# HJReachability/ilqgames

Hardware: AMD Instinct MI355X
Metric: iLQ iterations/sec (batch) (higher is better)
Workload: dtype f64

## Files before the change

### ilqgames_amd/csrc/ilqg_models.hpp

```cpp
#pragma once

#include "ilqg_common.hpp"
#include "ilqg_trig.hpp"

namespace ilqg {

template <typename T> __device__ __forceinline__ T t_sin(T x);
template <> __device__ __forceinline__ float t_sin<float>(float x) { return sinf(x); }
template <> __device__ __forceinline__ double t_sin<double>(double x) { return sin(x); }
template <typename T> __device__ __forceinline__ T t_cos(T x);
template <> __device__ __forceinline__ float t_cos<float>(float x) { return cosf(x); }
template <> __device__ __forceinline__ double t_cos<double>(double x) { return cos(x); }
template <typename T> __device__ __forceinline__ T t_tan(T x);
template <> __device__ __forceinline__ float t_tan<float>(float x) { return tanf(x); }
template <> __device__ __forceinline__ double t_tan<double>(double x) { return tan(x); }
template <typename T> __device__ __forceinline__ T t_sqrt(T x);
template <> __device__ __forceinline__ float t_sqrt<float>(float x) { return sqrtf(x); }
template <> __device__ __forceinline__ double t_sqrt<double>(double x) { return sqrt(x); }
template <typename T> __device__ __forceinline__ T t_hypot(T x, T y);
template <> __device__ __forceinline__ float t_hypot<float>(float x, float y) { return hypotf(x, y); }
template <> __device__ __forceinline__ double t_hypot<double>(double x, double y) { return hypot(x, y); }
template <typename T> __device__ __forceinline__ T t_abs(T x) { return x < T(0) ? -x : x; }

__device__ __forceinline__ bool is_unicycle(int kind) {
// ... 110 lines not shown
    xd[0] = L * t_cos(x[2]);
    xd[1] = L * t_sin(x[2]);
    xd[2] = x[3];
    xd[3] = u0;
    xd[4] = xd[5] = xd[6] = xd[7] = T(0);
  } else {
    sub_eval<T>(kind, L, x, u0, u1, xd, d0, d1);
    xd[6] = xd[7] = T(0);
  }
}
template <typename T>
__device__ __forceinline__ void sub_integrate8(int kind, T L, double interval, T* x, T u0, T u1, T d0 = T(0),
                                               T d1 = T(0)) {
  constexpr int XS = kSubStatesMax;
  const T h = T(interval / 2.0);
#pragma unroll 1
  for (int s = 0; s < 2; s++) {
    T k1[XS], k2[XS], k3[XS], k4[XS], xt[XS];
    sub_eval8(kind, L, x, u0, u1, k1, d0, d1);
#pragma unroll
    for (int i = 0; i < XS; i++) { k1[i] = h * k1[i]; xt[i] = x[i] + T(0.5) * k1[i]; }
    sub_eval8(kind, L, xt, u0, u1, k2, d0, d1);
#pragma unroll
    for (int i = 0; i < XS; i++) { k2[i] = h * k2[i]; xt[i] = x[i] + T(0.5) * k2[i]; }
    sub_eval8(kind, L, xt, u0, u1, k3, d0, d1);
#pragma unroll
    for (int i = 0; i < XS; i++) { k3[i] = h * k3[i]; xt[i] = x[i] + k3[i]; }
    sub_eval8(kind, L, xt, u0, u1, k4, d0, d1);
#pragma unroll
    for (int i = 0; i < XS; i++) {
      k4[i] = h * k4[i];
      x[i] += (k1[i] + T(2.0) * (k2[i] + k3[i]) + k4[i]) / T(6.0);
    }
  }
}

template <typename T> __device__ __forceinline__ void t_sincos(T x, T* s, T* c);
template <> __device__ __forceinline__ void t_sincos<float>(float x, float* s, float* c) { sincosf(x, s, c); }
template <> __device__ __forceinline__ void t_sincos<double>(double x, double* s, double* c) { sincos(x, s, c); }

template <typename T>
__device__ __forceinline__ T div_by(T x, T c, T rc) {
  const T q = x * rc;
  const T r = __builtin_fma(-q, c, x);
  return __builtin_fma(r, rc, q);
}
__device__ __forceinline__ float div_by(float x, float c, float rc) {
  const float q = x * rc;
  const float r = __builtin_fmaf(-q, c, x);
  return __builtin_fmaf(r, rc, q);
}

#pragma clang fp contract(off)
template <typename T, bool DIST = false, bool DUB = false>
__device__ __forceinline__ void sub_integrate_stages(int kind, T L, double interval, T* x, T u0, T u1, int q, int lane,
                                                     T* gth, bool any_car, T d0 = T(0), T d1 = T(0),
                                                     unsigned long long group = ~0ull) {
  const T h = T(interval / 2.0);
  const T six = T(6.0), rsix = T(1.0) / T(6.0), rL = T(1.0) / L;
  const bool dubins = DUB && kind == ILQG_DYN_DUBINS_CAR;
  const bool car = DIST ? false : (kind == ILQG_DYN_CAR_5D || kind == ILQG_DYN_CAR_6D);
  const bool car6 = car && kind == ILQG_DYN_CAR_6D;
  const int j = q & 3;
  const bool s1 = q >= 4;
  const T aj = j == 0 ? T(0) : (j == 3 ? T(1) : T(0.5));
  const T cq = aj + (s1 ? T(1) : T(0));
  const T ang0 = car ? x[3] : x[2];
  const T hk = h * u0;
  const T ang_q = t_fma(cq, hk, ang0);
  const T ang_end = t_fma(T(2), hk, ang0);
  const T v0 = car ? x[4] : x[3];
  const T hj = h * u1;
  T v_q, v_end, a_end = T(0);
  {
    const T a0 = x[5];
    const T a_1 = a0 + hj;
    const T v_1 = t_fma(T(0.5) * h, hj, t_fma(h, a0, v0));
    const T vb = s1 ? v_1 : v0, ab = s1 ? a_1 : a0;
    const T bj = j == 2 ? T(0.25) : (j == 3 ? T(0.5) : T(0));
    const T v6_q = t_fma(bj * h, hj, t_fma(aj * h, ab, vb));
    const T v6_end = t_fma(T(0.5) * h, hj, t_fma(h, a_1, v_1));
    const T v5_q = t_fma(cq, hj, v0), v5_end = t_fma(T(2), hj, v0);
    v_q = car6 ? v6_q : v5_q;
    v_end = car6 ? v6_end : v5_end;
    a_end = t_fma(T(2), hj, a0);
    if (dubins) v_q = L;
  }
  T th_q = ang_q, th_end = ang_end;
  if (any_car) {
    const T kth = car ? h * (div_by(v_q, L, rL) * fast_tan(ang_q, group)) : T(0);
    gth[lane] = kth;
    lds_sync(true);
    const T* g = gth + (lane & ~7);
    const T k0 = g[0], k1 = g[1], k2 = g[2], k3 = g[3], k4 = g[4], k5 = g[5], k6 = g[6], k7 = g[7];
    const T kprev = (lane & 7) ? gth[lane - 1] : T(0);
    const T th1 = x[2] + div_by(t_fma(T(2), k1 + k2, k0) + k3, six, rsix);
    const T th2 = th1 + div_by(t_fma(T(2), k5 + k6, k4) + k7, six, rsix);
    const T thb = s1 ? th1 : x[2];
    th_q = car ? t_fma(aj, kprev, thb) : ang_q;
    th_end = car ? th2 : ang_end;
  }
  T sn, cs;
  fast_sincos(th_q, &sn, &cs, group);
  const T kx = DIST ? h * t_fma(v_q, cs, d0) : h * (v_q * cs);
  const T ky = DIST ? h * t_fma(v_q, sn, d1) : h * (v_q * sn);
  T* gxy = gth + 64;
  gxy[2 * lane] = kx;
  gxy[2 * lane + 1] = ky;
  lds_sync(true);
  const T* gq = gxy + 2 * (lane & ~7);
  T px = x[0], py = x[1];
#pragma unroll
  for (int s = 0; s < 2; s++) {
    const T a1 = gq[8 * s + 0], b1 = gq[8 * s + 1], a2 = gq[8 * s + 2], b2 = gq[8 * s + 3];
    const T a3 = gq[8 * s + 4], b3 = gq[8 * s + 5], a4 = gq[8 * s + 6], b4 = gq[8 * s + 7];
    px += div_by(t_fma(T(2), a2 + a3, a1) + a4, six, rsix);
    py += div_by(t_fma(T(2), b2 + b3, b1) + b4, six, rsix);
  }
  x[0] = px;
  x[1] = py;
  x[2] = th_end;
  if (car) {
    x[3] = ang_end;
    x[4] = v_end;
    if (car6) x[5] = a_end;
  } else if (!dubins) {
    x[3] = v_end;
  }
}

template <typename T>
__device__ __forceinline__ T stage_value(T v) {
  asm volatile("" : "+v"(v));
  return v;
}

template <typename T, bool DUB = false>
__device__ __forceinline__ void sub_integrate_stages_seq(int kind, T L, double interval, T* x, T u0, T u1) {
  const T h = T(interval / 2.0);
  const T six = T(6.0), rsix = T(1.0) / T(6.0), rL = T(1.0) / L;
  const bool dubins = DUB && kind == ILQG_DYN_DUBINS_CAR;
  const bool car = kind == ILQG_DYN_CAR_5D || kind == ILQG_DYN_CAR_6D;
  const bool car6 = car && kind == ILQG_DYN_CAR_6D;
  const T ang0 = car ? x[3] : x[2];
  const T hk = h * u0;
  const T ang_end = t_fma(T(2), hk, ang0);
  const T v0 = car ? x[4] : x[3];
  const T hj = h * u1;
  const T a0 = x[5];
  const T a_1 = a0 + hj;
  const T v_1 = t_fma(T(0.5) * h, hj, t_fma(h, a0, v0));
  const T v6_end = t_fma(T(0.5) * h, hj, t_fma(h, a_1, v_1));
  const T v5_end = t_fma(T(2), hj, v0);
  const T v_end = car6 ? v6_end : v5_end;
  const T a_end = t_fma(T(2), hj, a0);
  T ang[8], vq[8], kth[8];
// ... 748 lines not shown
```

### ilqgames_amd/csrc/ilqg_solve.hpp

```cpp
#pragma once
#ifndef ILQG_ROLL_PRIO
#define ILQG_ROLL_PRIO 1
#endif

#include "ilqg_lq.hpp"
#include "ilqg_lq_openloop.hpp"
#include "ilqg_lq_feedback2.hpp"
#include "ilqg_lq_feedback1w.hpp"
#include "ilqg_lq_generic.hpp"
#include "ilqg_stages.hpp"

namespace ilqg {

template <typename T>
struct SolveArgs {
  const T* x0;
  T *xs, *us;
  T *P, *alpha;
  T* total_costs;
  int *iters, *status, *converged;
  const int* active;
  T* ws;
  size_t ws_stride;
  int fixed_iters;
// ... 610 lines not shown
    s = state_load<T>(w, L);
  }
  return s;
}

template <typename T>
__device__ __forceinline__ void trial_rollout_args(const SolveArgs<T>& sa, const InstanceBuffers<T>& ib, int b, int n,
                                                   SolveState<T>& s, RolloutArgs<T>& ra) {
  const int snew = 1 - s.sacc;
  ra.x0 = s.initial ? sa.x0 + size_t(b) * n : ib.XS(s.cur);
  ra.xs_ref = s.initial ? ib.XS(0) : ib.XS(s.cur);
  ra.us_ref = s.initial ? ib.US(0) : ib.US(s.cur);
  ra.P = s.initial ? ib.PB(0) : ib.PB(snew);
  ra.alpha = s.initial ? ib.AL(0) : ib.AL(snew);
  ra.alpha_scale = s.initial ? T(1) : s.step;
  ra.xs = s.initial ? ib.XS(1) : ib.XS(1 - s.cur);
  ra.us = s.initial ? ib.US(1) : ib.US(1 - s.cur);
  if (s.initial) {
    s.cur = 1;
    s.qmode = Q_COSTS;
  } else {
    s.qmode = sa.prm.linesearch ? Q_TRIAL : Q_LIN;
  }
}

template <typename T, int NX, int NP, int MU>
__device__ __forceinline__ void roll_pair_instances(const DevProblem& p, const SolveArgs<T>& sa, int b0, int b1, T* sm) {
  constexpr int n = NX, N = NP, m = NP * MU;
  const InstanceBuffers<T> ib0(p, sa, b0), ib1(p, sa, b1 < 0 ? b0 : b1);
  SolveState<T> s0, s1;
  RolloutArgs<T> r0, r1;
  auto enter = [&](const InstanceBuffers<T>& ib, int b, SolveState<T>& s, RolloutArgs<T>& r) -> bool {
    if (b < 0) return false;
    if (!sa.first) {
      if (reinterpret_cast<const SolveState<T>*>(ib.w + ib.L.state)->stage != ST_ROLLOUT) return false;
    } else if (sa.active && !sa.active[b]) {
      if (threadIdx.x == 0) reinterpret_cast<SolveState<T>*>(ib.w + ib.L.state)->stage = ST_DONE;
      return false;
    }
    s = trial_state_begin<T>(p, sa, ib, b, n, N, m);
    if (s.stage != ST_ROLLOUT) return false;
    trial_rollout_args<T>(sa, ib, b, n, s, r);
    r.iv = instance_values(p, b);
    return true;
  };
  const bool g0 = enter(ib0, b0, s0, r0), g1 = enter(ib1, b1, s1, r1);
  if (!g0 && !g1) return;
  __syncthreads();
  rollout_pair<T, NX, NP * MU, (MU == 1)>(p, g0 ? r0 : r1, g1 ? r1 : r0, g0, g1, sm, int(threadIdx.x));
  if (g0) state_store<T>(ib0.w, ib0.L, s0);
  if (g1) state_store<T>(ib1.w, ib1.L, s1);
}

template <typename T, int NX, int NP, int MU, int W, int PHASE = TRIAL_FUSED, int PROGID = 0, bool BOUND = (PROGID >= kBoundProg)>
__device__ __forceinline__ void trial_part_instance(const DevProblem& p, const short* maps,
                                                    const SolveArgs<T>& sa, int b, T* sm) {
  static_assert(PHASE == TRIAL_FUSED || W == 1, "the split phases run one wave per instance");
  static_assert(NX > 0 || PHASE != TRIAL_FUSED, "the run-time-dimensioned path (NX = 0) runs the split passes");
  const int n = NX > 0 ? NX : p.n, N = NX > 0 ? NP : p.N, m = NX > 0 ? NP * MU : p.m;
  const int Tn = p.T;
  const ilqg_solver_params& prm = sa.prm;
  const InstanceBuffers<T> ib(p, sa, b);
  const WsLayout& L = ib.L;
  T* const w = ib.w;
  int* const t_extreme = ib.t_extreme();
  T* const lambdas = w + L.lambdas;
  T* const costs = sa.total_costs + size_t(b) * N;
  const int t = threadIdx.x, wave = t >> 6, lane = t & 63;

  const size_t re = PHASE == TRIAL_DECIDE ? 0 : (rollout_lds_elems(n, m) + 3) & ~size_t(3);
  const size_t qe = trial_phase_quad_elems<T>(p, PHASE, sa.rows_cw, PROGID != 0 && PHASE == TRIAL_FUSED);
  constexpr int RW = W > 1 ? W - 1 : 1;
  const int rwave = W > 1 ? wave - 1 : 0;
  T* const sm_roll = sm;
  T* const sm_quad = sm + re + size_t(rwave < 0 ? 0 : rwave) * qe;
  T* const sm_quad0 = sm + re;
  int* const flags = reinterpret_cast<int*>(sm + re + size_t(RW) * qe);
  T* const ed_slot = reinterpret_cast<T*>(flags + 2);

  SolveState<T> s = trial_state_begin<T>(p, sa, ib, b, n, N, m);
  const int max_iters = solve_max_iters(sa);
  tl_stamp(sa.prof, b, 0, t == 0);
  const long long pr_start = clock64();
  long long qph[8] = {0, 0, 0, 0, 0, 0, 0, 0};
  long long rph[4] = {0, 0, 0, 0};

#pragma unroll 1
  while (s.stage == ST_ROLLOUT || s.stage == ST_QUAD) {
    __syncthreads();
    const bool roll = PHASE != TRIAL_DECIDE && s.stage == ST_ROLLOUT;
    RolloutArgs<T> ra;
    if (roll) {
      trial_rollout_args<T>(sa, ib, b, n, s, ra);
      if constexpr (BOUND || PHASE == TRIAL_ROLL) ra.iv = instance_values(p, b);
    }
    if (t == 0) {
      flags[0] = roll ? 0 : Tn;
      flags[1] = 0;
    }
    __syncthreads();
    tl_stamp(sa.prof, b, 1, t == 0);
    if (roll && wave == 0) {
#if ILQG_ROLL_PRIO
      __builtin_amdgcn_s_setprio(ILQG_ROLL_PRIO);
#endif
      if constexpr (NX > 0)
        rollout_instance<T, NX, NP * MU, (NX == 4 && NP == 2), (MU == 1), (NX == 3 && NP == 2 && MU == 1),
                         (NX == 4 * NP && MU == 2 && NP <= 2), dims_use_plain_rk4(NX, NP, MU)>(
                                         p, ra, sm_roll, lane, W > 1 ? &flags[0] : nullptr,
                                         (kProfile && sa.prof) ? rph : nullptr, kTimeline ? sa.prof : nullptr, b);
      else
        rollout_instance_rt<T>(p, ra, sm_roll, lane);
#if ILQG_ROLL_PRIO
      __builtin_amdgcn_s_setprio(0);
#endif
    }
    tl_stamp(sa.prof, b, 2, t == 0);
    if (roll && W == 1) {
      __syncthreads();
      if (t == 0) flags[0] = Tn;
      __syncthreads();
    }
    if (PHASE == TRIAL_ROLL) break;

    const int qmode = s.qmode;
    if constexpr (PHASE == TRIAL_FUSED) {
    QuadArgs<T> qa = trial_quad_args<T, BOUND>(p, ib, s, sa.compact != 0, b);
    qa.phacc = (kProfile && sa.prof) ? qph : nullptr;
    qa.tl = kTimeline ? sa.prof : nullptr;
    qa.tl_b = b;
    long long tq0 = (kProfile && sa.prof) ? clock64() : 0;
    static_assert(W <= 2, "the deferred forward pass reads the linearisation on the first row wave while no other row wave "
                          "may overwrite it yet: with more than one row wave set defer_forward = 0 or hold them back");
    if (s.ed_pending && rwave == 0) {
      LQArgs<T> fa{};
      fa.A = w + L.A;
      fa.scratch = w + L.lqscr;
      fa.x0 = nullptr;
      fa.dx = nullptr;
      fa.ed_out = ed_slot;
      fa.T_steps = Tn;
      if (sa.compact) {
        fa.compact = w + L.Q;
        fa.compact_tab = p.row_prog + p.rp_compact_off;
        fa.dt = p.dt;
      }
      constexpr int FWD_LDSE = 4 * 2 * ((NX * NX + LQCfg<T, NX, NP, MU>::SCR + 3) & ~3) + 2 * NX + 8;
      lq_forward_pass_body<T, NX, NP, MU, 64, FWD_LDSE>(fa, sm_quad, lane);
    }
    tl_stamp(sa.prof, b, 3, rwave == 0 && lane == 0);
    typedef typename RowProgSel<PROGID>::type RowProg;
    constexpr bool SHARE_LAST = PROGID != 0 && W == 2 && ProgInRegisters<RowProg>::value && rows_state_in_registers(NX, NP * MU);
    if constexpr (SHARE_LAST) {
      const int cw = sa.rows_cw;
      const int nchunks = (Tn + cw - 1) / cw;
      const int rem = Tn % cw;
      constexpr unsigned first_half = static_prog_pass_split<typename RowProg::S>();
      if (wave == 0) qa.tl = nullptr;
#pragma unroll 1
      for (int c = (wave == 0 ? nchunks - 1 : 0); c < nchunks; c++) {
        const int k0 = rem == 0 ? c * cw : (c == 0 ? 0 : rem + (c - 1) * cw);
// ... 285 lines not shown
```

### ilqgames_amd/csrc/ilqg_stages.hpp

```cpp
#pragma once

#include "ilqg_common.hpp"
#include "ilqg_models.hpp"

#ifndef ILQG_ROLLOUT_PAIRS
#define ILQG_ROLLOUT_PAIRS 1
#endif

namespace ilqg {

template <typename T>
struct RolloutArgs {
  const T* x0;
  const T* xs_ref;
  const T* us_ref;
  const T* P;
  const T* alpha;
  T alpha_scale;
  T* xs;
  T* us;
  const float* iv = nullptr;
};

__host__ __device__ inline int rollout_stage_elems(int n, int m) { return (m * n + 2 * m + n + 3) & ~3; }
constexpr int kRolloutGatherElems = 192;
__host__ __device__ inline int rollout_lds_elems(int n, int m) {
  return ((2 * n + m + 3) & ~3) + 2 * rollout_stage_elems(n, m) + kRolloutGatherElems;
}

__device__ __forceinline__ void progress_publish(int* flag, int value) {
  __hip_atomic_store(flag, value, __ATOMIC_RELEASE, __HIP_MEMORY_SCOPE_WORKGROUP);
}
__device__ __forceinline__ int progress_observe(int* flag) {
  return __hip_atomic_load(flag, __ATOMIC_ACQUIRE, __HIP_MEMORY_SCOPE_WORKGROUP);
}

__host__ __device__ constexpr bool dims_use_plain_rk4(int nx, int np, int mu) {
  return (nx == 17 && np == 3 && mu == 2) || (nx == 8 && np == 2 && mu == 1);
}
template <typename T, int CN = 0, int CM = 0, bool DIST = false, bool DUB = false, bool AIR = false, bool PM = false,
          bool GEN = false>
__device__ __forceinline__ void rollout_instance(const DevProblem& p, const RolloutArgs<T>& a, T* sm, int t,
                                                 int* ready = nullptr, long long* phacc = nullptr,
                                                 long long* tl = nullptr, int tl_b = 0) {
  const int n = CN > 0 ? CN : p.n, m = CM > 0 ? CM : p.m, N = p.N, Tn = p.T;
  constexpr int NT = 64;
  T* sx = sm;
  T* sdx = sx + n;
  T* su = sdx + n;
  T* stg = sm + ((2 * n + m + 3) & ~3);
  const int WP = rollout_stage_elems(n, m);
  constexpr int S = int(sizeof(T));
  auto issue = [&](int k, int buf) {
    T* d = stg + buf * WP;
    dma_g2l<NT, false>(a.P + size_t(k) * m * n, d, m * n * S, t);
    dma_g2l<NT, false>(a.alpha + size_t(k) * m, d + m * n, m * S, t);
    dma_g2l<NT, false>(a.us_ref + size_t(k) * m, d + m * n + m, m * S, t);
    dma_g2l<NT, false>(a.xs_ref + size_t(k) * n, d + m * n + 2 * m, n * S, t);
  };
  constexpr int XS = GEN ? kSubStatesMax : 6;
  T xj[XS];
  const int grp = t >> 3, q = t & 7;
  const bool integ = grp < N && t < 64;
  int kind = ILQG_DYN_UNICYCLE_4D, xo = 0, uo = 0, xd = 0;
  T Lp = T(1);
#pragma unroll
  for (int e = 0; e < XS; e++) xj[e] = T(0);
  if (integ) {
    kind = p.sub_kind[grp];
    xo = p.xoff[grp];
    uo = p.uoff[grp];
    xd = p.xoff[grp + 1] - xo;
    Lp = T(subsystem_param(p, a.iv, grp));
#pragma unroll
    for (int e = 0; e < XS; e++) xj[e] = (e < xd) ? a.x0[xo + e] : T(0);
  }
  const T air_vp = AIR ? T(subsystem_param(p, a.iv, 1)) : T(0);
  T* const gth = stg + 2 * WP;
  const bool any_car = __any(integ && (kind == ILQG_DYN_CAR_5D || kind == ILQG_DYN_CAR_6D));
  issue(0, 0);
  long long rc0 = (kProfile && phacc) ? clock64() : 0, rc1;
#define ILQG_RPH(i) do { if (kProfile && phacc) { __builtin_amdgcn_sched_barrier(0); rc1 = clock64(); __builtin_amdgcn_sched_barrier(0); phacc[i] += rc1 - rc0; rc0 = rc1; } } while (0)
#pragma unroll 1
  for (int k = 0; k < Tn; k++) {
    dma_wait();
    if (kTimeline && (k & 31) == 0) tl_stamp(tl, tl_b, 20 + (k >> 5), t == 0);
    if (ready) progress_publish(ready, k);
    const T* sP = stg + (k & 1) * WP;
    const T* sal = sP + m * n;
    const T* sur = sal + m;
    const T* sxr = sur + m;
    {
      T mine = xj[0];
#pragma unroll
      for (int e = 1; e < XS; e++) mine = (q == e) ? xj[e] : mine;
      if (integ && q < xd) {
        sdx[xo + q] = mine - sxr[xo + q];
        a.xs[size_t(k) * n + xo + q] = mine;
      }
    }
    lds_sync(NT <= 64);
    ILQG_RPH(0);
    if (t < m) {
      T s = T(0);
      if constexpr (CN > 0) {
        constexpr int CH = 8;
#pragma unroll
        for (int c0 = 0; c0 < CN; c0 += CH) {
          T pr[CH], dv[CH];
#pragma unroll
          for (int c = 0; c < CH; c++)
            if (c0 + c < CN) {
              pr[c] = sP[t + m * (c0 + c)];
              dv[c] = sdx[c0 + c];
            }
#pragma unroll
          for (int c = 0; c < CH; c++)
            if (c0 + c < CN) s = t_fma(pr[c], dv[c], s);
        }
      } else {
        for (int c = 0; c < n; c++) s = t_fma(sP[t + m * c], sdx[c], s);
      }
      const T u = t_fma(-a.alpha_scale, sal[t], sur[t] - s);
      su[t] = u;
      a.us[size_t(k) * m + t] = u;
    }
    lds_sync(NT <= 64);
    ILQG_RPH(1);
    if (k + 1 < Tn) issue(k + 1, (k + 1) & 1);
    if (t < 64 && k + 1 < Tn) {
      const T u0 = integ ? su[uo] : T(0), u1 = integ ? su[uo + 1] : T(0);
      if constexpr (GEN) {
        if (integ) sub_integrate8<T>(kind, Lp, p.dt, xj, u0, u1);
      } else if constexpr (AIR) {
        if (grp == 0) sub_integrate<T>(kind, Lp, p.dt, xj, u0, u1, air_vp);
      } else if constexpr (DIST) {
        const bool dist = integ && kind == ILQG_DYN_UNICYCLE_4D_DISTURBED;
        const T d0 = dist ? su[uo + 2] : T(0), d1 = dist ? su[uo + 3] : T(0);
        sub_integrate_stages<T, true>(kind, Lp, p.dt, xj, u0, u1, q, t, gth, false, d0, d1);
      } else if (PM && p.sub_kind[0] == ILQG_DYN_POINT_MASS_2D) {
        sub_integrate<T>(kind, Lp, p.dt, xj, u0, u1);
      } else {
        sub_integrate_stages<T, false, DUB>(kind, Lp, p.dt, xj, u0, u1, q, t, gth, any_car);
      }
    }
    ILQG_RPH(2);
  }
#undef ILQG_RPH
  if (ready) progress_publish(ready, Tn);
}

__host__ __device__ constexpr bool rollout_pairs(int nx, int np, int mu) {
  return nx > 0 && np <= 4 && np * mu <= 32 && !(nx == 4 && np == 2) && !(nx == 3 && np == 2 && mu == 1) &&
         !(nx == 4 * np && mu == 2 && np <= 2) && !dims_use_plain_rk4(nx, np, mu) && ILQG_ROLLOUT_PAIRS;
}
__host__ __device__ inline int rollout_pair_lds_elems(int n, int m) {
  return 2 * ((2 * n + m + 3) & ~3) + 4 * rollout_stage_elems(n, m) + kRolloutGatherElems;
}

template <int H>
__device__ __forceinline__ void dma_g2l_half(const void* g_, void* l, int nbytes, int tl) {
  const void* g = uniform_ptr(g_);
  for (int off = 0; off < nbytes; off += 128) {
    const int my = off + tl * 4;
    if (my < nbytes)
      __builtin_amdgcn_global_load_lds((glb_vptr)((const char*)g + unsigned(my)), (lds_vptr)((char*)l + off - 128 * H), 4, 0, 0);
  }
}

template <typename T, int CN, int CM, bool DUB>
__device__ __forceinline__ void rollout_pair(const DevProblem& p, const RolloutArgs<T>& a0, const RolloutArgs<T>& a1,
                                             bool act0, bool act1, T* sm, int t) {
  static_assert(CN > 0 && CM > 0 && CM <= 32, "compile-time dimensions");
  constexpr int n = CN, m = CM;
  const int N = p.N, Tn = p.T;
  const int h = t >> 5, tl = t & 31;
  constexpr int S0 = (2 * n + m + 3) & ~3;
  const int WP = rollout_stage_elems(n, m);
  T* const sx = sm + h * S0;
  T* const sdx = sx + n;
  T* const su = sdx + n;
  T* const stg = sm + 2 * S0 + h * 2 * WP;
  T* const gth = sm + 2 * S0 + 4 * WP;
  constexpr int S = int(sizeof(T));
  const bool act = h ? act1 : act0;
  auto issue = [&](int k, int buf) {
    if (h == 0) {
      T* d = sm + 2 * S0 + buf * WP;
      dma_g2l_half<0>(a0.P + size_t(k) * m * n, d, m * n * S, tl);
      dma_g2l_half<0>(a0.alpha + size_t(k) * m, d + m * n, m * S, tl);
      dma_g2l_half<0>(a0.us_ref + size_t(k) * m, d + m * n + m, m * S, tl);
      dma_g2l_half<0>(a0.xs_ref + size_t(k) * n, d + m * n + 2 * m, n * S, tl);
      asm volatile("; rollout_pair: lower half staged" ::: "memory");
    } else {
      T* d = sm + 2 * S0 + 2 * WP + buf * WP;
      dma_g2l_half<1>(a1.P + size_t(k) * m * n, d, m * n * S, tl);
// ... 19 lines not shown
  if (integ) {
    kind = p.sub_kind[grp];
    xo = p.xoff[grp];
    uo = p.uoff[grp];
    xd = p.xoff[grp + 1] - xo;
    Lp = T(subsystem_param(p, iv, grp));
#pragma unroll
    for (int e = 0; e < XS; e++) xj[e] = (e < xd) ? x0[xo + e] : T(0);
  }
  const bool any_car = __any(integ && (kind == ILQG_DYN_CAR_5D || kind == ILQG_DYN_CAR_6D));
  issue(0, 0);
#pragma unroll 1
  for (int k = 0; k < Tn; k++) {
    dma_wait();
    const T* sP = stg + (k & 1) * WP;
    const T* sal = sP + m * n;
    const T* sur = sal + m;
    const T* sxr = sur + m;
    {
      T mine = xj[0];
#pragma unroll
      for (int e = 1; e < XS; e++) mine = (q == e) ? xj[e] : mine;
      if (integ && q < xd) {
        sdx[xo + q] = mine - sxr[xo + q];
        if (act) xs_out[size_t(k) * n + xo + q] = mine;
      }
    }
    lds_sync(true);
    if (tl < m) {
      T s = T(0);
      constexpr int CH = 8;
#pragma unroll
      for (int c0 = 0; c0 < CN; c0 += CH) {
        T pr[CH], dv[CH];
#pragma unroll
        for (int c = 0; c < CH; c++)
          if (c0 + c < CN) {
            pr[c] = sP[tl + m * (c0 + c)];
            dv[c] = sdx[c0 + c];
          }
#pragma unroll
        for (int c = 0; c < CH; c++)
          if (c0 + c < CN) s = t_fma(pr[c], dv[c], s);
      }
      const T u = t_fma(-alpha_scale, sal[tl], sur[tl] - s);
      su[tl] = u;
      if (act) us_out[size_t(k) * m + tl] = u;
    }
    lds_sync(true);
    if (k + 1 < Tn) issue(k + 1, (k + 1) & 1);
    if (k + 1 < Tn) {
      const T u0 = integ ? su[uo] : T(0), u1 = integ ? su[uo + 1] : T(0);
      sub_integrate_stages<T, false, DUB>(kind, Lp, p.dt, xj, u0, u1, q, t, gth, any_car, T(0), T(0),
                                          h ? 0xffffffff00000000ull : 0x00000000ffffffffull);
    }
  }
}

__host__ __device__ constexpr int rollout_lanes_per_wave(int np) { return 64 / np; }
__host__ __device__ inline int rollout_lanes_dx_stride(int n) { return n | 1; }
__host__ __device__ inline int rollout_lanes_lds_elems(int n, int m, int np) {
  return 2 * rollout_stage_elems(n, m) + ((rollout_lanes_per_wave(np) * rollout_lanes_dx_stride(n) + 3) & ~3);
}

template <typename T, int CN, int CM, int NP, bool DUB>
__device__ __forceinline__ void rollout_lanes(const DevProblem& p, const RolloutArgs<T>& a, T step, T* xs_out, T* us_out,
                                              bool act, T* sm, int t) {
  static_assert(CN > 0 && CM > 0 && NP > 0, "compile-time dimensions");
  constexpr int n = CN, m = CM, MU = CM / NP, C = rollout_lanes_per_wave(NP);
  const int Tn = p.T;
  const int WP = rollout_stage_elems(n, m);
  T* const stg = sm;
  const int DS = rollout_lanes_dx_stride(n);
  const int c = t / NP, i = t - c * NP;
  const bool live = c < C;
  T* const sdx = sm + 2 * WP + (live ? c : 0) * DS;
  constexpr int S = int(sizeof(T));
  auto issue = [&](int k, int buf) {
    T* d = stg + buf * WP;
    dma_g2l<64, false>(a.P + size_t(k) * m * n, d, m * n * S, t);
    dma_g2l<64, false>(a.alpha + size_t(k) * m, d + m * n, m * S, t);
    dma_g2l<64, false>(a.us_ref + size_t(k) * m, d + m * n + m, m * S, t);
    dma_g2l<64, false>(a.xs_ref + size_t(k) * n, d + m * n + 2 * m, n * S, t);
  };
  constexpr int XS = 6;
  T xj[XS];
  const int kind = p.sub_kind[i];
  const int xo = p.xoff[i], uo = p.uoff[i], xd = p.xoff[i + 1] - xo, ud = p.udim[i];
  const T Lp = T(subsystem_param(p, a.iv, i));
#pragma unroll
  for (int e = 0; e < XS; e++) xj[e] = (e < xd) ? a.x0[xo + e] : T(0);
  const bool store = act && live;
  issue(0, 0);
#pragma unroll 1
  for (int k = 0; k < Tn; k++) {
    dma_wait();
    const T* sP = stg + (k & 1) * WP;
    const T* sal = sP + m * n;
    const T* sur = sal + m;
    const T* sxr = sur + m;
#pragma unroll
    for (int e = 0; e < XS; e++)
      if (e < xd) {
        if (live) sdx[xo + e] = xj[e] - sxr[xo + e];
        if (store) xs_out[size_t(k) * n + xo + e] = xj[e];
      }
    lds_sync(true);
// ... 336 lines not shown
```

### ilqgames_amd/csrc/ilqg_trig.hpp

```cpp
#pragma once

#include <hip/hip_runtime.h>

#pragma clang fp contract(off)

namespace ilqg {

constexpr double kTrigFastLimit = 1.0e9;
constexpr float kTrigFastLimitF = 2.0e3f;

__host__ __device__ __forceinline__ int trig_reduce(double x, double* r) {
  const double n = __builtin_rint(x * 0x1.45f306dc9c883p-1);
  double t = __builtin_fma(-n, 0x1.921fb54442d18p+0, x);
  t = __builtin_fma(-n, 0x1.1a62633145c07p-54, t);
  t = __builtin_fma(-n, -0x1.f1976b7ed8fbcp-110, t);
  *r = t;
  return int(n);
}
__host__ __device__ __forceinline__ int trig_reduce(float x, float* r) {
  const float n = __builtin_rintf(x * 0.6366197466850281f);
  float t = __builtin_fmaf(-n, 1.5707963705062866f, x);
  t = __builtin_fmaf(-n, -4.371138828673793e-08f, t);
  t = __builtin_fmaf(-n, -1.7151245100058819e-15f, t);
  *r = t;
  return int(n);
}

__host__ __device__ __forceinline__ void trig_kernels(double r, double* s, double* c) {
  const double z = r * r;
  double ps = __builtin_fma(z, 1.58969099521155010221e-10, -2.50507602534068634195e-08);
  double pc = __builtin_fma(z, -1.13596475577881948265e-11, 2.08757232129817482790e-09);
  ps = __builtin_fma(z, ps, 2.75573137070700676789e-06);
  pc = __builtin_fma(z, pc, -2.75573143513906633035e-07);
  ps = __builtin_fma(z, ps, -1.98412698298579493134e-04);
  pc = __builtin_fma(z, pc, 2.48015872894767294178e-05);
  ps = __builtin_fma(z, ps, 8.33333333332248946124e-03);
  pc = __builtin_fma(z, pc, -1.38888888888741095749e-03);
  ps = __builtin_fma(z, ps, -1.66666666666666324348e-01);
  pc = __builtin_fma(z, pc, 4.16666666666666019037e-02);
  *s = __builtin_fma(r * z, ps, r);
  const double hz = 0.5 * z, w = 1.0 - hz;
  *c = w + __builtin_fma(z * z, pc, (1.0 - w) - hz);
}
__host__ __device__ __forceinline__ void trig_kernels(float r, float* s, float* c) {
  const float z = r * r;
  float ps = __builtin_fmaf(z, 2.7183114939898219064e-06f, -1.98393348360966317347e-04f);
  float pc = __builtin_fmaf(z, 2.43904487962774090654e-05f, -1.38867637746099294692e-03f);
  ps = __builtin_fmaf(z, ps, 8.3333293858894631756e-03f);
  pc = __builtin_fmaf(z, pc, 4.16666233237390631894e-02f);
  ps = __builtin_fmaf(z, ps, -1.66666666416265235595e-01f);
  pc = __builtin_fmaf(z, pc, -4.99999997251031003120e-01f);
  *s = __builtin_fmaf(r * z, ps, r);
  *c = __builtin_fmaf(z, pc, 1.0f);
}

template <typename T>
__host__ __device__ __forceinline__ void fast_sincos_core(T x, T* s, T* c) {
  T r, sr, cr;
  const int n = trig_reduce(x, &r);
  trig_kernels(r, &sr, &cr);
  const bool swap = n & 1;
  const T sv = swap ? cr : sr, cv = swap ? sr : cr;
  *s = (n & 2) ? -sv : sv;
  *c = ((n + 1) & 2) ? -cv : cv;
}

#if defined(__HIP_DEVICE_COMPILE__)
__device__ __forceinline__ bool trig_group_any(bool mine, unsigned long long group) {
  if (group == ~0ull) return __any(mine);
  return (__ballot(mine) & group) != 0;
}
#endif

__host__ __device__ __forceinline__ unsigned long long trig_mulhi64(unsigned long long a, unsigned long long b) {
#if defined(__HIP_DEVICE_COMPILE__)
  return __umul64hi(a, b);
#else
  return (unsigned long long)(((unsigned __int128)a * b) >> 64);
#endif
}
__host__ __device__ inline int trig_reduce_large(double x, double* r_hi, double* r_lo) {
  const unsigned long long two_over_pi[20] = {
      0x0000000000000000ull, 0xa2f9836e4e441529ull, 0xfc2757d1f534ddc0ull, 0xdb6295993c439041ull,
      0xfe5163abdebbc561ull, 0xb7246e3a424dd2e0ull, 0x06492eea09d1921cull, 0xfe1deb1cb129a73eull,
      0xe88235f52ebb4484ull, 0xe99c7026b45f7e41ull, 0x3991d639835339f4ull, 0x9c845f8bbdf9283bull,
      0x1ff897ffde05980full, 0xef2f118b5a0a6d1full, 0x6d367ecf27cb09b7ull, 0x4f463f669e5fea2dull,
      0x7527bac7ebe5f17bull, 0x3d0739f78a5292eaull, 0x6bfb5fb11f8d5d08ull, 0x56033046fc7b6babull};
  const unsigned long long ux = (unsigned long long)__builtin_bit_cast(long long, x) & 0x7fffffffffffffffull;
  const int E = int(ux >> 52) - 1023;
  const unsigned long long m = (ux & 0x000fffffffffffffull) | 0x0010000000000000ull;
  const int pos = E + 10;
  const int w = pos >> 6, sh = pos & 63;
  const unsigned long long t0 = two_over_pi[w], t1 = two_over_pi[w + 1], t2 = two_over_pi[w + 2], t3 = two_over_pi[w + 3];
  const unsigned long long W2 = sh ? (t0 << sh) | (t1 >> (64 - sh)) : t0;
  const unsigned long long W1 = sh ? (t1 << sh) | (t2 >> (64 - sh)) : t1;
  const unsigned long long W0 = sh ? (t2 << sh) | (t3 >> (64 - sh)) : t2;
  const unsigned long long p0 = m * W0;
  const unsigned long long c0 = trig_mulhi64(m, W0);
  const unsigned long long l1 = m * W1;
  const unsigned long long p1 = l1 + c0;
  const unsigned long long c1 = trig_mulhi64(m, W1) + (p1 < l1 ? 1ull : 0ull);
  const unsigned long long p2 = m * W2 + c1;
  int q = int(p2 >> 62);
  unsigned long long fh = (p2 << 2) | (p1 >> 62), fl = (p1 << 2) | (p0 >> 62);
  const bool neg = (fh >> 63) != 0;
  if (neg) {
    q += 1;
    fl = ~fl + 1ull;
    fh = ~fh + (fl == 0 ? 1ull : 0ull);
  }
  int shift = 0;
  if (fh == 0) {
    fh = fl;
// ... 7 lines not shown
  }
  const int lz = __builtin_clzll(fh);
  const unsigned long long nh = lz ? (fh << lz) | (fl >> (64 - lz)) : fh, nl = fl << lz;
  shift += lz;
  const double a = double((long long)(nh >> 11)), b = double((long long)(((nh & 0x7ffull) << 42) | (nl >> 22)));
  double f_hi = __builtin_ldexp(a, 75 - 128 - shift), f_lo = __builtin_ldexp(b, 22 - 128 - shift);
  if (neg) {
    f_hi = -f_hi;
    f_lo = -f_lo;
  }
  const double pio2_hi = 0x1.921fb54442d18p+0, pio2_lo = 0x1.1a62633145c07p-54;
  const double rh = f_hi * pio2_hi;
  *r_lo = __builtin_fma(f_hi, pio2_hi, -rh) + __builtin_fma(f_hi, pio2_lo, f_lo * pio2_hi);
  *r_hi = rh;
  return q & 3;
}

constexpr double kTrigMidLimit = 0x1p47;
__host__ __device__ __forceinline__ int trig_reduce_mid(double x, double* r) {
  const double n = __builtin_rint(x * 0x1.45f306dc9c883p-1);
  double t = __builtin_fma(-n, 0x1.921fb54442d18p+0, x);
  t = __builtin_fma(-n, 0x1.1a62633145c07p-54, t);
  t = __builtin_fma(-n, -0x1.f1976b7ed8fbcp-110, t);
  *r = t;
  return int(n - 4.0 * __builtin_rint(0.25 * n));
}

__host__ __device__ inline void large_sincos(double x, double* s, double* c) {
  if (__builtin_fabs(x) <= kTrigMidLimit) {
    double r, sr, cr;
    const int n = trig_reduce_mid(x, &r);
    trig_kernels(r, &sr, &cr);
    const bool swap = n & 1;
    const double sv = swap ? cr : sr, cv = swap ? sr : cr;
    *s = (n & 2) ? -sv : sv;
    *c = ((n + 1) & 2) ? -cv : cv;
    return;
  }
  if (!(__builtin_fabs(x) < __builtin_inf())) {
    *s = *c = x - x;
    return;
  }
  double rh, rl, sr, cr;
  const int n = trig_reduce_large(x, &rh, &rl);
  trig_kernels(rh, &sr, &cr);
  const double s1 = __builtin_fma(rl, cr, sr), c1 = __builtin_fma(-rl, sr, cr);
  const bool swap = n & 1;
  const double sv = swap ? c1 : s1, cv = swap ? s1 : c1;
  const double sa = (n & 2) ? -sv : sv;
  *s = x < 0.0 ? -sa : sa;
  *c = ((n + 1) & 2) ? -cv : cv;
}

__host__ __device__ __forceinline__ void fast_sincos(double x, double* s, double* c, unsigned long long group = ~0ull) {
  const bool mine = !(__builtin_fabs(x) <= kTrigFastLimit);
#if defined(__HIP_DEVICE_COMPILE__)
  const bool any = trig_group_any(mine, group);
#else
  const bool any = mine;
  (void)group;
#endif
  if (__builtin_expect(any, 0)) {
    if (mine) {
      large_sincos(x, s, c);
      return;
    }
  }
  fast_sincos_core<double>(x, s, c);
}
__host__ __device__ __forceinline__ void fast_sincos(float x, float* s, float* c, unsigned long long group = ~0ull) {
  const bool mine = !(__builtin_fabsf(x) <= kTrigFastLimitF);
#if defined(__HIP_DEVICE_COMPILE__)
  const bool any = trig_group_any(mine, group);
#else
  const bool any = mine;
  (void)group;
#endif
  if (__builtin_expect(any, 0)) {
    if (mine) {
      double sd, cd;
      large_sincos(double(x), &sd, &cd);
      *s = float(sd);
      *c = float(cd);
      return;
    }
  }
  fast_sincos_core<float>(x, s, c);
}

__host__ __device__ __forceinline__ double trig_div(double a, double b) {
#if defined(__HIP_DEVICE_COMPILE__)
  double rc = __builtin_amdgcn_rcp(b);
#else
  double rc = double(1.0f / float(b));
#endif
  rc = __builtin_fma(__builtin_fma(-b, rc, 1.0), rc, rc);
  rc = __builtin_fma(__builtin_fma(-b, rc, 1.0), rc, rc);
  const double q = a * rc;
  return __builtin_fma(__builtin_fma(-q, b, a), rc, q);
}
__host__ __device__ __forceinline__ float trig_div(float a, float b) {
#if defined(__HIP_DEVICE_COMPILE__)
  float rc = __builtin_amdgcn_rcpf(b);
#else
  float rc = 1.0f / b;
#endif
  rc = __builtin_fmaf(__builtin_fmaf(-b, rc, 1.0f), rc, rc);
  const float q = a * rc;
  return __builtin_fmaf(__builtin_fmaf(-q, b, a), rc, q);
}
template <typename T>
__host__ __device__ __forceinline__ T fast_tan_core(T x) {
  T r, sr, cr;
  const int n = trig_reduce(x, &r);
  trig_kernels(r, &sr, &cr);
  const bool odd = n & 1;
  return trig_div(odd ? -cr : sr, odd ? sr : cr);
}
__host__ __device__ inline double large_tan(double x) {
  if (__builtin_fabs(x) <= kTrigMidLimit) {
    double r, sr, cr;
    const int n = trig_reduce_mid(x, &r);
    trig_kernels(r, &sr, &cr);
    const bool odd = n & 1;
    return trig_div(odd ? -cr : sr, odd ? sr : cr);
  }
  double s, c;
  large_sincos(x, &s, &c);
  return s / c;
}
__host__ __device__ __forceinline__ double fast_tan(double x, unsigned long long group = ~0ull) {
  const bool mine = !(__builtin_fabs(x) <= kTrigFastLimit);
#if defined(__HIP_DEVICE_COMPILE__)
  const bool any = trig_group_any(mine, group);
#else
  const bool any = mine;
  (void)group;
#endif
  if (__builtin_expect(any, 0)) {
    if (mine) return large_tan(x);
  }
  return fast_tan_core<double>(x);
}
__host__ __device__ __forceinline__ float fast_tan(float x, unsigned long long group = ~0ull) {
  const bool mine = !(__builtin_fabsf(x) <= kTrigFastLimitF);
#if defined(__HIP_DEVICE_COMPILE__)
  const bool any = trig_group_any(mine, group);
#else
  const bool any = mine;
  (void)group;
#endif
  if (__builtin_expect(any, 0)) {
    if (mine) return float(large_tan(double(x)));
  }
  return fast_tan_core<float>(x);
}

}

#pragma clang fp contract(fast)
```

Measured before the change: 2.107 million.

## Tune rollout register use: inline-asm trig chains, wave-level LDS DMA, lane-select tweaks

Adds a ROOM template flag to the rollout. The trig polynomial evaluation becomes hand-written interleaved v_fma_f64 chains that take SGPR constants. The per-stage P/alpha/us/xs staging now uses a per-wave global_load_lds helper that pairs the alpha and us_ref loads. Lane indices are pinned in VGPRs through an empty asm barrier, and a few branches are replaced by selects (an unconditional LDS read for kprev, unguarded u loads). The aim is to cut register pressure and instruction count in the fused rollout loop. In exchange it constrains compiler scheduling and depends on hand asm. For f64 the new path is only enabled for one specific problem shape with a nonzero program id.

```diff
diff --git a/ilqgames_amd/csrc/ilqg_models.hpp b/ilqgames_amd/csrc/ilqg_models.hpp
--- a/ilqgames_amd/csrc/ilqg_models.hpp
+++ b/ilqgames_amd/csrc/ilqg_models.hpp
@@ -186,10 +186,10 @@
 }
 
 #pragma clang fp contract(off)
-template <typename T, bool DIST = false, bool DUB = false>
+template <typename T, bool DIST = false, bool DUB = false, bool CHAINS = true>
 __device__ __forceinline__ void sub_integrate_stages(int kind, T L, double interval, T* x, T u0, T u1, int q, int lane,
-                                                     T* gth, bool any_car, T d0 = T(0), T d1 = T(0),
-                                                     unsigned long long group = ~0ull) {
+                                                     T* gth, bool any_car, T d0, T d1, unsigned long long group,
+                                                     int qsel) {
   const T h = T(interval / 2.0);
   const T six = T(6.0), rsix = T(1.0) / T(6.0), rL = T(1.0) / L;
   const bool dubins = DUB && kind == ILQG_DYN_DUBINS_CAR;
@@ -210,7 +210,8 @@
     const T a0 = x[5];
     const T a_1 = a0 + hj;
     const T v_1 = t_fma(T(0.5) * h, hj, t_fma(h, a0, v0));
-    const T vb = s1 ? v_1 : v0, ab = s1 ? a_1 : a0;
+    const bool s1v = qsel >= 4;
+    const T vb = s1v ? v_1 : v0, ab = s1v ? a_1 : a0;
     const T bj = j == 2 ? T(0.25) : (j == 3 ? T(0.5) : T(0));
     const T v6_q = t_fma(bj * h, hj, t_fma(aj * h, ab, vb));
     const T v6_end = t_fma(T(0.5) * h, hj, t_fma(h, a_1, v_1));
@@ -222,20 +223,21 @@
   }
   T th_q = ang_q, th_end = ang_end;
   if (any_car) {
-    const T kth = car ? h * (div_by(v_q, L, rL) * fast_tan(ang_q, group)) : T(0);
+    const T kth = car ? h * (div_by(v_q, L, rL) * fast_tan<CHAINS>(ang_q, group)) : T(0);
     gth[lane] = kth;
     lds_sync(true);
     const T* g = gth + (lane & ~7);
     const T k0 = g[0], k1 = g[1], k2 = g[2], k3 = g[3], k4 = g[4], k5 = g[5], k6 = g[6], k7 = g[7];
-    const T kprev = (lane & 7) ? gth[lane - 1] : T(0);
+    const T kread = gth[lane - 1];
+    const T kprev = qsel ? kread : T(0);
     const T th1 = x[2] + div_by(t_fma(T(2), k1 + k2, k0) + k3, six, rsix);
     const T th2 = th1 + div_by(t_fma(T(2), k5 + k6, k4) + k7, six, rsix);
-    const T thb = s1 ? th1 : x[2];
+    const T thb = (qsel >= 4) ? th1 : x[2];
     th_q = car ? t_fma(aj, kprev, thb) : ang_q;
     th_end = car ? th2 : ang_end;
   }
   T sn, cs;
-  fast_sincos(th_q, &sn, &cs, group);
+  fast_sincos<CHAINS>(th_q, &sn, &cs, group);
   const T kx = DIST ? h * t_fma(v_q, cs, d0) : h * (v_q * cs);
   const T ky = DIST ? h * t_fma(v_q, sn, d1) : h * (v_q * sn);
   T* gxy = gth + 64;
diff --git a/ilqgames_amd/csrc/ilqg_solve.hpp b/ilqgames_amd/csrc/ilqg_solve.hpp
--- a/ilqgames_amd/csrc/ilqg_solve.hpp
+++ b/ilqgames_amd/csrc/ilqg_solve.hpp
@@ -686,6 +686,10 @@
   if (g1) state_store<T>(ib1.w, ib1.L, s1);
 }
 
+__host__ __device__ constexpr bool fused_rollout_room(int elem_bytes, int nx, int np, int mu, int progid) {
+  return elem_bytes == 4 || (progid != 0 && nx == 14 && np == 3 && mu == 2);
+}
+
 template <typename T, int NX, int NP, int MU, int W, int PHASE = TRIAL_FUSED, int PROGID = 0, bool BOUND = (PROGID >= kBoundProg)>
 __device__ __forceinline__ void trial_part_instance(const DevProblem& p, const short* maps,
                                                     const SolveArgs<T>& sa, int b, T* sm) {
@@ -740,7 +744,8 @@
 #endif
       if constexpr (NX > 0)
         rollout_instance<T, NX, NP * MU, (NX == 4 && NP == 2), (MU == 1), (NX == 3 && NP == 2 && MU == 1),
-                         (NX == 4 * NP && MU == 2 && NP <= 2), dims_use_plain_rk4(NX, NP, MU)>(
+                         (NX == 4 * NP && MU == 2 && NP <= 2), dims_use_plain_rk4(NX, NP, MU),
+                         fused_rollout_room(int(sizeof(T)), NX, NP, MU, PROGID)>(
                                          p, ra, sm_roll, lane, W > 1 ? &flags[0] : nullptr,
                                          (kProfile && sa.prof) ? rph : nullptr, kTimeline ? sa.prof : nullptr, b);
       else
diff --git a/ilqgames_amd/csrc/ilqg_stages.hpp b/ilqgames_amd/csrc/ilqg_stages.hpp
--- a/ilqgames_amd/csrc/ilqg_stages.hpp
+++ b/ilqgames_amd/csrc/ilqg_stages.hpp
@@ -38,8 +38,21 @@
 __host__ __device__ constexpr bool dims_use_plain_rk4(int nx, int np, int mu) {
   return (nx == 17 && np == 3 && mu == 2) || (nx == 8 && np == 2 && mu == 1);
 }
+__device__ __forceinline__ void dma_g2l_wave(const void* g_, void* l, int nbytes, int lane, const void* g2_ = nullptr,
+                                             void* l2 = nullptr) {
+  const char* g = (const char*)uniform_ptr(g_);
+  const char* g2 = g2_ ? (const char*)uniform_ptr(g2_) : nullptr;
+  const unsigned voff = unsigned(lane) << 2;
+  for (int off = 0; off < nbytes; off += 256) {
+    if (off + 256 <= nbytes || lane < ((nbytes - off) >> 2)) {
+      __builtin_amdgcn_global_load_lds((glb_vptr)((g + off) + voff), (lds_vptr)((char*)l + off), 4, 0, 0);
+      if (g2) __builtin_amdgcn_global_load_lds((glb_vptr)((g2 + off) + voff), (lds_vptr)((char*)l2 + off), 4, 0, 0);
+    }
+  }
+}
+
 template <typename T, int CN = 0, int CM = 0, bool DIST = false, bool DUB = false, bool AIR = false, bool PM = false,
-          bool GEN = false>
+          bool GEN = false, bool ROOM = true>
 __device__ __forceinline__ void rollout_instance(const DevProblem& p, const RolloutArgs<T>& a, T* sm, int t,
                                                  int* ready = nullptr, long long* phacc = nullptr,
                                                  long long* tl = nullptr, int tl_b = 0) {
@@ -51,12 +64,11 @@
   T* stg = sm + ((2 * n + m + 3) & ~3);
   const int WP = rollout_stage_elems(n, m);
   constexpr int S = int(sizeof(T));
-  auto issue = [&](int k, int buf) {
+  auto issue = [&](int k, int buf, int ln) {
     T* d = stg + buf * WP;
-    dma_g2l<NT, false>(a.P + size_t(k) * m * n, d, m * n * S, t);
-    dma_g2l<NT, false>(a.alpha + size_t(k) * m, d + m * n, m * S, t);
-    dma_g2l<NT, false>(a.us_ref + size_t(k) * m, d + m * n + m, m * S, t);
-    dma_g2l<NT, false>(a.xs_ref + size_t(k) * n, d + m * n + 2 * m, n * S, t);
+    dma_g2l_wave(a.P + size_t(k) * m * n, d, m * n * S, ln);
+    dma_g2l_wave(a.alpha + size_t(k) * m, d + m * n, m * S, ln, a.us_ref + size_t(k) * m, d + m * n + m);
+    dma_g2l_wave(a.xs_ref + size_t(k) * n, d + m * n + 2 * m, n * S, ln);
   };
   constexpr int XS = GEN ? kSubStatesMax : 6;
   T xj[XS];
@@ -78,12 +90,14 @@
   const T air_vp = AIR ? T(subsystem_param(p, a.iv, 1)) : T(0);
   T* const gth = stg + 2 * WP;
   const bool any_car = __any(integ && (kind == ILQG_DYN_CAR_5D || kind == ILQG_DYN_CAR_6D));
-  issue(0, 0);
+  issue(0, 0, t);
+  int qv = q, tv = t;
   long long rc0 = (kProfile && phacc) ? clock64() : 0, rc1;
 #define ILQG_RPH(i) do { if (kProfile && phacc) { __builtin_amdgcn_sched_barrier(0); rc1 = clock64(); __builtin_amdgcn_sched_barrier(0); phacc[i] += rc1 - rc0; rc0 = rc1; } } while (0)
 #pragma unroll 1
   for (int k = 0; k < Tn; k++) {
     dma_wait();
+    if constexpr (ROOM) asm volatile("" : "+v"(qv), "+v"(tv));
     if (kTimeline && (k & 31) == 0) tl_stamp(tl, tl_b, 20 + (k >> 5), t == 0);
     if (ready) progress_publish(ready, k);
     const T* sP = stg + (k & 1) * WP;
@@ -93,7 +107,7 @@
     {
       T mine = xj[0];
 #pragma unroll
-      for (int e = 1; e < XS; e++) mine = (q == e) ? xj[e] : mine;
+      for (int e = 1; e < XS; e++) mine = (qv == e) ? xj[e] : mine;
       if (integ && q < xd) {
         sdx[xo + q] = mine - sxr[xo + q];
         a.xs[size_t(k) * n + xo + q] = mine;
@@ -101,7 +115,7 @@
     }
     lds_sync(NT <= 64);
     ILQG_RPH(0);
-    if (t < m) {
+    if (tv < m) {
       T s = T(0);
       if constexpr (CN > 0) {
         constexpr int CH = 8;
@@ -127,9 +141,9 @@
     }
     lds_sync(NT <= 64);
     ILQG_RPH(1);
-    if (k + 1 < Tn) issue(k + 1, (k + 1) & 1);
+    if (k + 1 < Tn) issue(k + 1, (k + 1) & 1, tv);
     if (t < 64 && k + 1 < Tn) {
-      const T u0 = integ ? su[uo] : T(0), u1 = integ ? su[uo + 1] : T(0);
+      const T u0 = su[uo], u1 = su[uo + 1];
       if constexpr (GEN) {
         if (integ) sub_integrate8<T>(kind, Lp, p.dt, xj, u0, u1);
       } else if constexpr (AIR) {
@@ -137,11 +151,11 @@
       } else if constexpr (DIST) {
         const bool dist = integ && kind == ILQG_DYN_UNICYCLE_4D_DISTURBED;
         const T d0 = dist ? su[uo + 2] : T(0), d1 = dist ? su[uo + 3] : T(0);
-        sub_integrate_stages<T, true>(kind, Lp, p.dt, xj, u0, u1, q, t, gth, false, d0, d1);
+        sub_integrate_stages<T, true, false, ROOM>(kind, Lp, p.dt, xj, u0, u1, q, t, gth, false, d0, d1, ~0ull, qv);
       } else if (PM && p.sub_kind[0] == ILQG_DYN_POINT_MASS_2D) {
         sub_integrate<T>(kind, Lp, p.dt, xj, u0, u1);
       } else {
-        sub_integrate_stages<T, false, DUB>(kind, Lp, p.dt, xj, u0, u1, q, t, gth, any_car);
+        sub_integrate_stages<T, false, DUB, ROOM>(kind, Lp, p.dt, xj, u0, u1, q, t, gth, any_car, T(0), T(0), ~0ull, qv);
       }
     }
     ILQG_RPH(2);
@@ -267,7 +281,7 @@
     if (k + 1 < Tn) {
       const T u0 = integ ? su[uo] : T(0), u1 = integ ? su[uo + 1] : T(0);
       sub_integrate_stages<T, false, DUB>(kind, Lp, p.dt, xj, u0, u1, q, t, gth, any_car, T(0), T(0),
-                                          h ? 0xffffffff00000000ull : 0x00000000ffffffffull);
+                                          h ? 0xffffffff00000000ull : 0x00000000ffffffffull, q);
     }
   }
 }
diff --git a/ilqgames_amd/csrc/ilqg_trig.hpp b/ilqgames_amd/csrc/ilqg_trig.hpp
--- a/ilqgames_amd/csrc/ilqg_trig.hpp
+++ b/ilqgames_amd/csrc/ilqg_trig.hpp
@@ -26,22 +26,65 @@
   return int(n);
 }
 
+__host__ __device__ __forceinline__ void trig_poly_chains(double z, double* ps, double* pc) {
+  constexpr double S2 = -1.66666666666666324348e-01, S3 = 8.33333333332248946124e-03, S4 = -1.98412698298579493134e-04,
+                   S5 = 2.75573137070700676789e-06, S6 = -2.50507602534068634195e-08, S7 = 1.58969099521155010221e-10;
+  constexpr double C2 = 4.16666666666666019037e-02, C3 = -1.38888888888741095749e-03, C4 = 2.48015872894767294178e-05,
+                   C5 = -2.75573143513906633035e-07, C6 = 2.08757232129817482790e-09, C7 = -1.13596475577881948265e-11;
+#if defined(__HIP_DEVICE_COMPILE__)
+  double s, c;
+  asm("v_fma_f64 %0, %2, %3, %4\n\t"
+      "v_fma_f64 %1, %2, %5, %6\n\t"
+      "v_fma_f64 %0, %2, %0, %7\n\t"
+      "v_fma_f64 %1, %2, %1, %8\n\t"
+      "v_fma_f64 %0, %2, %0, %9\n\t"
+      "v_fma_f64 %1, %2, %1, %10\n\t"
+      "v_fma_f64 %0, %2, %0, %11\n\t"
+      "v_fma_f64 %1, %2, %1, %12\n\t"
+      "v_fma_f64 %0, %2, %0, %13\n\t"
+      "v_fma_f64 %1, %2, %1, %14"
+      : "=&v"(s), "=&v"(c)
+      : "v"(z), "s"(S7), "v"(S6), "s"(C7), "v"(C6), "v"(S5), "v"(C5), "v"(S4), "v"(C4), "v"(S3), "v"(C3), "v"(S2), "v"(C2));
+  *ps = s;
+  *pc = c;
+#else
+  double s = __builtin_fma(z, S7, S6), c = __builtin_fma(z, C7, C6);
+  s = __builtin_fma(z, s, S5);
+  c = __builtin_fma(z, c, C5);
+  s = __builtin_fma(z, s, S4);
+  c = __builtin_fma(z, c, C4);
+  s = __builtin_fma(z, s, S3);
+  c = __builtin_fma(z, c, C3);
+  s = __builtin_fma(z, s, S2);
+  c = __builtin_fma(z, c, C2);
+  *ps = s;
+  *pc = c;
+#endif
+}
+
+template <bool CHAINS = false>
 __host__ __device__ __forceinline__ void trig_kernels(double r, double* s, double* c) {
   const double z = r * r;
-  double ps = __builtin_fma(z, 1.58969099521155010221e-10, -2.50507602534068634195e-08);
-  double pc = __builtin_fma(z, -1.13596475577881948265e-11, 2.08757232129817482790e-09);
-  ps = __builtin_fma(z, ps, 2.75573137070700676789e-06);
-  pc = __builtin_fma(z, pc, -2.75573143513906633035e-07);
-  ps = __builtin_fma(z, ps, -1.98412698298579493134e-04);
-  pc = __builtin_fma(z, pc, 2.48015872894767294178e-05);
-  ps = __builtin_fma(z, ps, 8.33333333332248946124e-03);
-  pc = __builtin_fma(z, pc, -1.38888888888741095749e-03);
-  ps = __builtin_fma(z, ps, -1.66666666666666324348e-01);
-  pc = __builtin_fma(z, pc, 4.16666666666666019037e-02);
+  double ps, pc;
+  if constexpr (CHAINS) {
+    trig_poly_chains(z, &ps, &pc);
+  } else {
+    ps = __builtin_fma(z, 1.58969099521155010221e-10, -2.50507602534068634195e-08);
+    pc = __builtin_fma(z, -1.13596475577881948265e-11, 2.08757232129817482790e-09);
+    ps = __builtin_fma(z, ps, 2.75573137070700676789e-06);
+    pc = __builtin_fma(z, pc, -2.75573143513906633035e-07);
+    ps = __builtin_fma(z, ps, -1.98412698298579493134e-04);
+    pc = __builtin_fma(z, pc, 2.48015872894767294178e-05);
+    ps = __builtin_fma(z, ps, 8.33333333332248946124e-03);
+    pc = __builtin_fma(z, pc, -1.38888888888741095749e-03);
+    ps = __builtin_fma(z, ps, -1.66666666666666324348e-01);
+    pc = __builtin_fma(z, pc, 4.16666666666666019037e-02);
+  }
   *s = __builtin_fma(r * z, ps, r);
   const double hz = 0.5 * z, w = 1.0 - hz;
   *c = w + __builtin_fma(z * z, pc, (1.0 - w) - hz);
 }
+template <bool CHAINS = false>
 __host__ __device__ __forceinline__ void trig_kernels(float r, float* s, float* c) {
   const float z = r * r;
   float ps = __builtin_fmaf(z, 2.7183114939898219064e-06f, -1.98393348360966317347e-04f);
@@ -54,11 +97,11 @@
   *c = __builtin_fmaf(z, pc, 1.0f);
 }
 
-template <typename T>
+template <typename T, bool CHAINS = false>
 __host__ __device__ __forceinline__ void fast_sincos_core(T x, T* s, T* c) {
   T r, sr, cr;
   const int n = trig_reduce(x, &r);
-  trig_kernels(r, &sr, &cr);
+  trig_kernels<CHAINS>(r, &sr, &cr);
   const bool swap = n & 1;
   const T sv = swap ? cr : sr, cv = swap ? sr : cr;
   *s = (n & 2) ? -sv : sv;
@@ -172,6 +215,7 @@
   *c = ((n + 1) & 2) ? -cv : cv;
 }
 
+template <bool CHAINS = false>
 __host__ __device__ __forceinline__ void fast_sincos(double x, double* s, double* c, unsigned long long group = ~0ull) {
   const bool mine = !(__builtin_fabs(x) <= kTrigFastLimit);
 #if defined(__HIP_DEVICE_COMPILE__)
@@ -186,8 +230,9 @@
       return;
     }
   }
-  fast_sincos_core<double>(x, s, c);
-}
+  fast_sincos_core<double, CHAINS>(x, s, c);
+}
+template <bool CHAINS = false>
 __host__ __device__ __forceinline__ void fast_sincos(float x, float* s, float* c, unsigned long long group = ~0ull) {
   const bool mine = !(__builtin_fabsf(x) <= kTrigFastLimitF);
 #if defined(__HIP_DEVICE_COMPILE__)
@@ -229,11 +274,11 @@
   const float q = a * rc;
   return __builtin_fmaf(__builtin_fmaf(-q, b, a), rc, q);
 }
-template <typename T>
+template <typename T, bool CHAINS = false>
 __host__ __device__ __forceinline__ T fast_tan_core(T x) {
   T r, sr, cr;
   const int n = trig_reduce(x, &r);
-  trig_kernels(r, &sr, &cr);
+  trig_kernels<CHAINS>(r, &sr, &cr);
   const bool odd = n & 1;
   return trig_div(odd ? -cr : sr, odd ? sr : cr);
 }
@@ -249,6 +294,7 @@
   large_sincos(x, &s, &c);
   return s / c;
 }
+template <bool CHAINS = false>
 __host__ __device__ __forceinline__ double fast_tan(double x, unsigned long long group = ~0ull) {
   const bool mine = !(__builtin_fabs(x) <= kTrigFastLimit);
 #if defined(__HIP_DEVICE_COMPILE__)
@@ -260,8 +306,9 @@
   if (__builtin_expect(any, 0)) {
     if (mine) return large_tan(x);
   }
-  return fast_tan_core<double>(x);
-}
+  return fast_tan_core<double, CHAINS>(x);
+}
+template <bool CHAINS = false>
 __host__ __device__ __forceinline__ float fast_tan(float x, unsigned long long group = ~0ull) {
   const bool mine = !(__builtin_fabsf(x) <= kTrigFastLimitF);
 #if defined(__HIP_DEVICE_COMPILE__)
```

Result: faster. 2.140 million, median of 6 (+1.6%).
